# SysCV/LiDAR_snow_sim

Measured on NVIDIA H100. Metric: augmented LiDAR points/sec, higher is better.
Workload: dtype f64

## Files before the change

include/lidar_snow_sim.h:

```cpp
#ifndef LIDAR_SNOW_SIM_H
#define LIDAR_SNOW_SIM_H

#include <stdint.h>

#ifdef __cplusplus
extern "C" {
#endif

#if defined(__GNUC__)
#define LSS_API __attribute__((visibility("default")))
#else
#define LSS_API
#endif

typedef struct lss_engine lss_engine;

typedef enum {
    LSS_OK = 0,
    LSS_ERR_INVALID_ARG = 1,
    LSS_ERR_CUDA = 2,
    LSS_ERR_NO_TABLE = 3,
    LSS_ERR_RANGE_INDEX = 4,
    LSS_ERR_NEGATIVE_INTENSITY = 5,
    LSS_ERR_OCCLUDER_OVERFLOW = 6,
// ... 31 lines not shown
                                       int n_azimuth_buckets, void *stream, int *table_id_out);
LSS_API lss_status lss_free_particles(lss_engine *e, int table_id);
LSS_API lss_status lss_table_info(lss_engine *e, int table_id, int64_t *n_particles, int64_t *n_entries, int64_t *bytes);

LSS_API lss_status lss_snowfall_batch(lss_engine *e, int table_id, const float *d_points, const int64_t *h_cloud_offsets,
                              int n_clouds, const int32_t *h_order, double beam_divergence_deg, const float *d_theta,
                              const double *h_thresh_poly, const double *h_plane_in, const int32_t *h_ymins_in,
                              double noise_floor, uint32_t flags, float *d_out_points,
                              int32_t *d_out_counts, double *d_out_stats, float *d_out_full, int32_t *d_out_perm,
                              int32_t *d_out_nocc, void *d_workspace, int64_t workspace_bytes, void *stream);
LSS_API lss_status lss_snowfall_batch_slots(lss_engine *e, int table_id, const float *d_points,
                                            const int64_t *h_cloud_offsets, const int32_t *d_cloud_counts, int n_clouds,
                                            const int32_t *h_order, double beam_divergence_deg, const float *d_theta,
                                            const double *h_thresh_poly, const double *h_plane_in,
                                            const int32_t *h_ymins_in, double noise_floor, uint32_t flags,
                                            float *d_out_points, int32_t *d_out_counts, double *d_out_stats,
                                            float *d_out_full, int32_t *d_out_perm, int32_t *d_out_nocc,
                                            void *d_workspace, int64_t workspace_bytes, void *stream);
LSS_API int64_t lss_snowfall_workspace_bytes(int64_t n_total, int n_clouds);
LSS_API lss_status lss_snowfall_batch_host(lss_engine *e, int table_id, const float *h_points,
                                           const int64_t *h_cloud_offsets, int n_clouds, const int32_t *h_order,
                                           double beam_divergence_deg, const double *h_thresh_poly, double noise_floor,
                                           uint32_t flags, int n_chunks, float *h_out_points, int32_t *h_out_counts,
                                           double *h_out_stats);
LSS_API lss_status lss_snowfall_batch_host_submit(lss_engine *e, int table_id, const float *h_points,
                                                  const int64_t *h_cloud_offsets, int n_clouds, const int32_t *h_order,
                                                  double beam_divergence_deg, const double *h_thresh_poly,
                                                  double noise_floor, uint32_t flags, int n_chunks, float *h_out_points,
                                                  int32_t *h_out_counts, double *h_out_stats, int *ticket_out);
LSS_API lss_status lss_snowfall_batch_host_wait(lss_engine *e, int ticket);
LSS_API int lss_host_pipe_trace(lss_engine *e, float *out, int cap_chunks);
LSS_API lss_status lss_check_async(lss_engine *e, void *stream);
LSS_API int64_t lss_launch_count(const lss_engine *e);
LSS_API lss_status lss_noise_threshold_poly(lss_engine *e, const float *d_points, const int64_t *h_cloud_offsets,
                                    int n_clouds, double noise_floor, const double *h_plane_in,
                                    const int32_t *h_ymins_in, double *d_poly_out, double *d_plane_out,
                                    double *d_fit_out, int32_t *d_ymins_out, void *d_workspace,
                                    int64_t workspace_bytes, void *stream);
LSS_API int64_t lss_prepass_workspace_bytes(int64_t n_total, int n_clouds);

LSS_API lss_status lss_wet_ground_batch(lss_engine *e, const float *d_points, const int64_t *h_cloud_offsets,
                                const int32_t *d_cloud_counts, int n_clouds, double water_height, double pavement_depth,
                                double noise_floor, double power_factor, int flat_earth, double delta, int replace,
                                const double *h_plane_in, const int32_t *h_ymins_in, float *d_out_points,
                                double *d_out_intensity64, int32_t *d_out_counts, int32_t *d_out_passthrough,
                                double *d_out_plane, double *d_out_fit, int32_t *d_out_ymins, void *d_workspace,
                                int64_t workspace_bytes, void *stream);
LSS_API lss_status lss_wet_ground_batch_params(lss_engine *e, const float *d_points, const int64_t *h_cloud_offsets,
                                               const int32_t *d_cloud_counts, int n_clouds,
                                               const double *h_water_height, double pavement_depth,
                                               double noise_floor, double power_factor, int flat_earth, double delta,
                                               int replace, const double *h_plane_in, const int32_t *h_ymins_in,
                                               float *d_out_points, double *d_out_intensity64, int32_t *d_out_counts,
                                               int32_t *d_out_passthrough, double *d_out_plane, double *d_out_fit,
                                               int32_t *d_out_ymins, void *d_workspace, int64_t workspace_bytes,
                                               void *stream);
LSS_API int64_t lss_wet_ground_workspace_bytes(int64_t n_total, int n_clouds);
LSS_API lss_status lss_wet_ground_batch_poly(lss_engine *e, const float *d_points, const int64_t *h_cloud_offsets,
                                             const int32_t *d_cloud_counts, int n_clouds, const double *h_water_height,
                                             double pavement_depth, double noise_floor, double power_factor,
                                             int flat_earth, double delta, int replace, const double *h_plane_in,
                                             const int32_t *h_ymins_in, const uint32_t *h_mt_state,
                                             float *d_out_points, double *d_out_intensity64, int32_t *d_out_counts,
                                             int32_t *d_out_passthrough, double *d_out_plane, double *d_out_fit,
                                             int32_t *d_out_ymins, uint32_t *d_mt_state_out, double *d_out_poly_fit,
                                             void *d_workspace, int64_t workspace_bytes, void *stream);
// ... 219 lines not shown
```

lidar_snow_sim_b200/_lib.py:

```python
import ctypes
import os

_HERE = os.path.dirname(os.path.abspath(__file__))
LIB_PATH = os.path.join(_HERE, 'liblss_b200.so')

LSS_OK = 0
LSS_ERR_INVALID_ARG = 1
LSS_ERR_CUDA = 2
LSS_ERR_NO_TABLE = 3
LSS_ERR_RANGE_INDEX = 4
LSS_ERR_NEGATIVE_INTENSITY = 5
LSS_ERR_OCCLUDER_OVERFLOW = 6
LSS_ERR_WORKSPACE = 7
LSS_ERR_NO_SENSOR = 8
LSS_ERR_TOO_FEW_GROUND = 9
LSS_ERR_INTENSITY_RANGE = 10

FLAG_THRESHOLD_FILTER = 0x1
FLAG_CAMERA_FOV = 0x2
FLAG_DEVICE_PREPASS = 0x4
FLAG_ASSUME_SORTED = 0x8
FOG_HARD, FOG_SOFT, FOG_GAIN = 0x1, 0x2, 0x4
DROR_CUBE, DROR_WORK_STATS = 0x1, 0x100

# ... 17 lines not shown
    LSS_ERR_TOO_FEW_GROUND: TypeError,
    LSS_ERR_INTENSITY_RANGE: ValueError,
}

_c = ctypes
_P = ctypes.c_void_p
SIGNATURES = [
    ('lss_create', _c.c_int, [_c.c_int, _c.POINTER(_P)]),
    ('lss_destroy', None, [_P]),
    ('lss_status_string', _c.c_char_p, [_c.c_int]),
    ('lss_last_error', _c.c_char_p, [_P]),
    ('lss_version', _c.c_int, []),
    ('lss_set_sensor', _c.c_int, [_P, _c.c_int, _P, _P, _P, _P]),
    ('lss_set_camera', _c.c_int, [_P, _P, _P, _P, _c.c_int, _c.c_int]),
    ('lss_upload_particles', _c.c_int, [_P, _c.c_int, _P, _P, _c.c_double, _c.c_int, _P, _c.POINTER(_c.c_int)]),
    ('lss_upload_particles_device', _c.c_int, [_P, _c.c_int, _P, _P, _c.c_double, _c.c_int, _P,
                                               _c.POINTER(_c.c_int)]),
    ('lss_free_particles', _c.c_int, [_P, _c.c_int]),
    ('lss_table_info', _c.c_int, [_P, _c.c_int, _c.POINTER(_c.c_int64), _c.POINTER(_c.c_int64),
                                  _c.POINTER(_c.c_int64)]),
    ('lss_snowfall_batch', _c.c_int, [_P, _c.c_int, _P, _P, _c.c_int, _P, _c.c_double, _P, _P, _P, _P, _c.c_double,
                                      _c.c_uint32, _P, _P, _P, _P, _P, _P, _P, _c.c_int64, _P]),
    ('lss_snowfall_batch_slots', _c.c_int, [_P, _c.c_int, _P, _P, _P, _c.c_int, _P, _c.c_double, _P, _P, _P, _P,
                                            _c.c_double, _c.c_uint32, _P, _P, _P, _P, _P, _P, _P, _c.c_int64, _P]),
    ('lss_snowfall_workspace_bytes', _c.c_int64, [_c.c_int64, _c.c_int]),
    ('lss_host_pipe_trace', _c.c_int, [_P, _P, _c.c_int]),
    ('lss_snowfall_batch_host', _c.c_int, [_P, _c.c_int, _P, _P, _c.c_int, _P, _c.c_double, _P, _c.c_double, _c.c_uint32,
                                           _c.c_int, _P, _P, _P]),
    ('lss_snowfall_batch_host_submit', _c.c_int, [_P, _c.c_int, _P, _P, _c.c_int, _P, _c.c_double, _P, _c.c_double,
                                                  _c.c_uint32, _c.c_int, _P, _P, _P, _c.POINTER(_c.c_int)]),
    ('lss_snowfall_batch_host_wait', _c.c_int, [_P, _c.c_int]),
    ('lss_check_async', _c.c_int, [_P, _P]),
    ('lss_launch_count', _c.c_int64, [_P]),
    ('lss_debug_range_grid', _c.c_int, [_P]),
    ('lss_debug_azimuth', _c.c_int, [_P, _P, _P, _c.c_int64, _P, _P]),
    ('lss_debug_solve_phases', _c.c_int, [_P, _c.c_int, _P, _c.c_int]),
    ('lss_noise_threshold_poly', _c.c_int, [_P, _P, _P, _c.c_int, _c.c_double, _P, _P, _P, _P, _P, _P, _P, _c.c_int64,
                                            _P]),
    ('lss_prepass_workspace_bytes', _c.c_int64, [_c.c_int64, _c.c_int]),
    ('lss_wet_ground_batch', _c.c_int, [_P, _P, _P, _P, _c.c_int, _c.c_double, _c.c_double, _c.c_double, _c.c_double,
                                        _c.c_int, _c.c_double, _c.c_int, _P, _P, _P, _P, _P, _P, _P, _P, _P, _P,
                                        _c.c_int64, _P]),
    ('lss_wet_ground_batch_params', _c.c_int, [_P, _P, _P, _P, _c.c_int, _P, _c.c_double, _c.c_double, _c.c_double,
                                               _c.c_int, _c.c_double, _c.c_int, _P, _P, _P, _P, _P, _P, _P, _P, _P,
                                               _P, _c.c_int64, _P]),
    ('lss_wet_ground_workspace_bytes', _c.c_int64, [_c.c_int64, _c.c_int]),
    ('lss_wet_ground_batch_poly', _c.c_int, [_P, _P, _P, _P, _c.c_int, _P, _c.c_double, _c.c_double, _c.c_double,
                                             _c.c_int, _c.c_double, _c.c_int, _P, _P, _P, _P, _P, _P, _P, _P, _P, _P,
                                             _P, _P, _P, _c.c_int64, _P]),
    ('lss_wet_ground_poly_workspace_bytes', _c.c_int64, [_c.c_int64, _c.c_int]),
    ('lss_fog_batch', _c.c_int, [_P, _P, _c.c_int, _P, _c.c_int, _c.c_double, _c.c_double, _c.c_double, _P, _c.c_uint32,
                                 _c.c_int, _c.c_int, _P, _P, _P, _P, _P, _P, _P, _c.c_int64, _P]),
    ('lss_fog_workspace_bytes', _c.c_int64, [_c.c_int64, _c.c_int]),
    ('lss_fog_batch_params', _c.c_int, [_P, _P, _c.c_int, _P, _c.c_int, _P, _P, _P, _P, _P, _c.c_int, _c.c_uint32,
                                        _c.c_int, _c.c_int, _P, _P, _P, _P, _P, _P, _P, _c.c_int64, _P]),
    ('lss_fog_batch_params_workspace_bytes', _c.c_int64, [_c.c_int64, _c.c_int]),
    ('lss_fog_integral_tables', _c.c_int, [_P, _P, _c.c_int, _P, _P, _c.c_int64, _P]),
    ('lss_fog_integral_tables_workspace_bytes', _c.c_int64, [_c.c_int, _c.c_int]),
    ('lss_mie_tables', _c.c_int, [_P, _P, _P, _c.c_int, _P, _c.c_int, _P, _P, _c.c_int64, _P]),
    ('lss_mie_tables_workspace_bytes', _c.c_int64, [_P, _P, _c.c_int, _P, _c.c_int]),
    ('lss_lisa_batch', _c.c_int, [_P, _P, _c.c_int, _c.c_int64, _c.c_double, _c.c_int, _c.c_double, _c.c_double, _c.c_double,
                                  _c.c_double, _c.c_double, _c.c_double, _c.c_int, _P, _c.c_int, _c.c_uint64, _P, _P]),
    ('lss_lisa_cloud_batch', _c.c_int, [_P, _P, _c.c_int, _P, _P, _c.c_int, _P, _P, _P, _P, _c.c_int, _c.c_double,
                                        _c.c_double, _c.c_double, _c.c_double, _c.c_double, _c.c_int, _P, _c.c_int, _P, _P,
                                        _P, _P, _c.c_int64, _P]),
    ('lss_lisa_cloud_batch_workspace_bytes', _c.c_int64, [_c.c_int64, _c.c_int]),
# ... 56 lines not shown
                                            _c.c_int64, _P, _c.c_int]),
    ('lss_sample_particles', _c.c_int, [_P, _c.c_int, _c.c_double, _c.c_double, _c.c_double, _c.c_int, _c.c_uint64,
                                        _c.c_int64, _P, _c.c_int64, _P, _P, _P, _c.c_int64, _P]),
    ('lss_sample_particles_workspace_bytes', _c.c_int64, [_c.c_int, _c.c_int64]),
    ('lss_set_profiling', _c.c_int, [_P, _c.c_int]),
    ('lss_kernel_times', _c.c_int, [_P, _c.c_int, _P, _P, _c.c_int]),
    ('lss_kernel_name', _c.c_char_p, [_c.c_int]),
]

_lib = None


def load():
    global _lib
    if _lib is not None:
        return _lib
    if not os.path.exists(LIB_PATH):
        raise ImportError(f'{LIB_PATH} not found: build it with `python -m lidar_snow_sim_b200.build` '
                          f'(or __graft_entry__.build()); this engine has no CPU fallback')
    lib = ctypes.CDLL(LIB_PATH)
    for name, res, args in SIGNATURES:
        fn = getattr(lib, name)
        fn.restype = res
        fn.argtypes = args
    _lib = lib
    return lib


def check(status, engine_handle=None):
    if status == LSS_OK:
        return
    lib = load()
    msg = lib.lss_status_string(status).decode()
    if engine_handle:
        detail = lib.lss_last_error(engine_handle).decode()
        if detail:
            msg = f'{msg}: {detail}'
    raise _EXC.get(status, RuntimeError)(msg)
```

lidar_snow_sim_b200/csrc/api.cu:

```cuda
#include "common.cuh"
#include <cmath>
#include <cstring>
#include <cstdlib>

namespace {

void host_range_grid(double *R)
{
    const double stop = 120 + 299792458.0 * 1e-8;
    const double step = stop / (LSS_M_EXT - 1);
    for (int k = 0; k < LSS_M_EXT; k++) {
        double v = (k == LSS_M_EXT - 1) ? stop : k * step;
        R[k] = std::nearbyint(v * 100.0) / 100.0;
    }
}

void host_phase_table(const double *R, double *tab )
{
    const long double ctau = (long double)(299792458.0 * 1e-8);
    const long double pi = 3.14159265358979323846264338327950288L;
    for (int k = 0; k < LSS_M_EXT; k++) {
        const long double a = fmodl((long double)R[k] / ctau, 2.0L);
        tab[2 * k] = (double)sinl(pi * a);
        tab[2 * k + 1] = (double)cosl(pi * a);
    }
}

}

extern "C" {

int lss_version(void) { return 100; }

const char *lss_status_string(lss_status s)
{
    switch (s) {
        case LSS_OK: return "ok";
        case LSS_ERR_INVALID_ARG: return "invalid argument";
        case LSS_ERR_CUDA: return "CUDA error";
        case LSS_ERR_NO_TABLE: return "particle table set not found";
        case LSS_ERR_RANGE_INDEX: return "waveform index out of range (return beyond ~120 m on an occluded beam)";
        case LSS_ERR_NEGATIVE_INTENSITY: return "new intensity is negative";
        case LSS_ERR_OCCLUDER_OVERFLOW: return "too many occluders on one beam";
        case LSS_ERR_WORKSPACE: return "workspace too small";
        case LSS_ERR_NO_SENSOR: return "sensor / camera constants not set";
        case LSS_ERR_TOO_FEW_GROUND: return "fewer than 3 ground points: laser parameters cannot be estimated";
        case LSS_ERR_INTENSITY_RANGE:
            return "intensity histogram range (5, max(I/cos)) of the ground points is not finite or max is below 5";
    }
    return "unknown status";
}

const char *lss_last_error(const lss_engine *e) { return e ? e->last_error.c_str() : "null engine"; }

lss_status lss_create(int device, lss_engine **out)
{
    if (!out) return LSS_ERR_INVALID_ARG;
    *out = nullptr;
    int n_dev = 0;
    if (cudaGetDeviceCount(&n_dev) != cudaSuccess || n_dev == 0) return LSS_ERR_CUDA;
    if (device < 0 || device >= n_dev) return LSS_ERR_INVALID_ARG;
    lss_engine *e = new lss_engine();
    e->device = device;
    DeviceGuard g(device);
    double R[LSS_M_EXT];
    host_range_grid(R);
    std::vector<double> wtab(2 * LSS_M_EXT);
    host_phase_table(R, wtab.data());
    int zero = 0;
    cudaDeviceGetAttribute(&e->n_sm, cudaDevAttrMultiProcessorCount, device);
    if (e->n_sm <= 0) e->n_sm = 132;
    if (cudaMalloc(&e->d_R, sizeof(R)) != cudaSuccess || cudaMalloc(&e->d_status, sizeof(int)) != cudaSuccess ||
        cudaMalloc(&e->d_wtab, sizeof(double) * wtab.size()) != cudaSuccess ||
        cudaMemcpy(e->d_wtab, wtab.data(), sizeof(double) * wtab.size(), cudaMemcpyHostToDevice) != cudaSuccess ||
        cudaMalloc(&e->d_sensor, sizeof(SensorConst)) != cudaSuccess ||
        cudaMalloc(&e->d_camera, sizeof(CameraConst)) != cudaSuccess ||
        cudaMemcpy(e->d_R, R, sizeof(R), cudaMemcpyHostToDevice) != cudaSuccess ||
        cudaMemcpy(e->d_status, &zero, sizeof(int), cudaMemcpyHostToDevice) != cudaSuccess) {
        lss_destroy(e);
        return LSS_ERR_CUDA;
    }
    *out = e;
    return LSS_OK;
}

void lss_destroy(lss_engine *e)
{
    if (!e) return;
    DeviceGuard g(e->device);
    for (auto &kv : e->tables) {
        cudaFree(kv.second.d_rec);
        cudaFree(kv.second.d_tan);
        cudaFree(kv.second.d_plane_off);
        cudaFree(kv.second.d_entries);
        cudaFree(kv.second.d_bucket_start);
    }
    cudaFree(e->d_R);
    cudaFree(e->d_wtab);
    cudaFree(e->d_status);
    cudaFree(e->d_sensor);
    cudaFree(e->d_camera);
    lss_host_pipe_free(e);
    for (cudaStream_t st : e->side) if (st) { cudaStreamSynchronize(st); cudaStreamDestroy(st); }
    for (cudaEvent_t ev : e->side_ev) if (ev) cudaEventDestroy(ev);
    for (auto &sl : e->stage) {
        if (sl.done) { cudaEventSynchronize(sl.done); cudaEventDestroy(sl.done); }
        if (sl.host) cudaFreeHost(sl.host);
    }
    delete e;
}

// ... 289 lines not shown
```

lidar_snow_sim_b200/csrc/common.cuh:

```cuda
#pragma once
#include <cuda_runtime.h>
#include <stdint.h>
#include <stdio.h>
#include <string>
#include <vector>
#include <cstring>
#include <map>
#include <utility>

#include "../../include/lidar_snow_sim.h"

#define LSS_PI 3.141592653589793
#define LSS_TWO_PI 6.283185307179586
#define LSS_M_EXT 1230
#define LSS_ANG_MARGIN 1e-5

struct ParticleRec {
    double phi;
    double rho;
    double alpha;
};
struct ParticleTan {
    double t_right, t_left;
};
// ... 248 lines not shown
       LSS_K_FOG = 6, LSS_K_SCAN = 7, LSS_K_SOLVE = 8, LSS_K_VOXEL = 9, LSS_K_DROR = 10, LSS_K_LISA = 11,
       LSS_K_FOG_LUT = 12, LSS_K_MIE = 13, LSS_K_SELECT = 14, LSS_K_PA = 15, LSS_K_COUNT = 16 };

struct KernelTimer {
    lss_engine *e; cudaStream_t s; int idx = -1;
    KernelTimer(lss_engine *e_, int kernel, cudaStream_t s_) : e(e_), s(s_) {
        if (!e->profiling) return;
        lss_engine::TimedLaunch t; t.kernel = kernel;
        cudaEventCreate(&t.beg); cudaEventCreate(&t.end);
        cudaEventRecord(t.beg, s);
        e->timed.push_back(t); idx = (int)e->timed.size() - 1;
    }
    ~KernelTimer() { if (idx >= 0) cudaEventRecord(e->timed[idx].end, s); }
};

#define LSS_CUDA_CHECK(e, call)                                                                          \
    do {                                                                                                 \
        cudaError_t _err = (call);                                                                       \
        if (_err != cudaSuccess) {                                                                       \
            char _buf[512];                                                                              \
            snprintf(_buf, sizeof(_buf), "%s failed: %s (%s:%d)", #call, cudaGetErrorString(_err),      \
                     __FILE__, __LINE__);                                                                \
            (e)->last_error = _buf;                                                                      \
            return LSS_ERR_CUDA;                                                                         \
        }                                                                                                \
    } while (0)

struct DeviceGuard {
    int prev = -1;
    explicit DeviceGuard(int dev) { cudaGetDevice(&prev); if (prev != dev) cudaSetDevice(dev); else prev = -1; }
    ~DeviceGuard() { if (prev >= 0) cudaSetDevice(prev); }
};

static inline lss_status lss_fail(lss_engine *e, lss_status s, const char *msg)
{
    if (e) e->last_error = msg;
    return s;
}

struct BatchGeometry {
    int64_t n = 0, max_n = 0;
    std::vector<int32_t> tile_base;
};

inline lss_status lss_batch_geometry(lss_engine *e, const int64_t *h_cloud_offsets, int n_clouds, int tile,
                                     BatchGeometry &g)
{
    if (!h_cloud_offsets || n_clouds < 0) return lss_fail(e, LSS_ERR_INVALID_ARG, "null argument");
    if (n_clouds > 65535) return lss_fail(e, LSS_ERR_INVALID_ARG, "at most 65535 clouds per call");
    if (h_cloud_offsets[0] != 0) return lss_fail(e, LSS_ERR_INVALID_ARG, "cloud_offsets[0] must be 0");
    g.max_n = 0;
    g.tile_base.assign(tile > 0 ? n_clouds + 1 : 0, 0);
    for (int b = 0; b < n_clouds; b++) {
        const int64_t n = h_cloud_offsets[b + 1] - h_cloud_offsets[b];
        if (n < 0) return lss_fail(e, LSS_ERR_INVALID_ARG, "cloud_offsets must be non-decreasing");
        if (n >= (1LL << 31)) return lss_fail(e, LSS_ERR_INVALID_ARG, "cloud too large");
        g.max_n = n > g.max_n ? n : g.max_n;
        if (tile > 0) g.tile_base[b + 1] = g.tile_base[b] + (int32_t)((n + tile - 1) / tile);
    }
    g.n = h_cloud_offsets[n_clouds];
    return LSS_OK;
}

lss_status lss_build_tables(lss_engine *e, TableSet &ts, const double *d_xyr, const int64_t *h_plane_offsets,
                            cudaStream_t stream);
struct SnowfallArgs {
// ... 82 lines not shown
```

lidar_snow_sim_b200/csrc/solve.cu:

```cuda
#include "beam.cuh"

namespace {

constexpr int SOLVE_TPB = 128;
constexpr int SOLVE_WARPS = SOLVE_TPB / 32;
#ifndef LSS_SOLVE_CTAS
#define LSS_SOLVE_CTAS 5
#endif
#ifndef LSS_SOLVE_ARENA
#define LSS_SOLVE_ARENA 160
#endif
constexpr int SOLVE_CTAS_PER_SM = LSS_SOLVE_CTAS;
constexpr int ARENA = LSS_SOLVE_ARENA;
constexpr int SOLVE_LCAP = 128;
static_assert(SOLVE_LCAP + 1 <= ARENA, "a beam with SOLVE_LCAP occluders must fit a round of the arena on its own");
constexpr unsigned FULL = 0xffffffffu;

struct Beam {
    double d, right, left;
    bool straddle;
};

__device__ __forceinline__ void beam_limits(float th32, double half_div, Beam &bm)
{
    const double thd = (double)th32;
    double right = thd - half_div, left = thd + half_div;
    if (right < 0) right += LSS_TWO_PI;
    if (left < 0) left += LSS_TWO_PI;
    if (right > LSS_TWO_PI) right -= LSS_TWO_PI;
    if (left > LSS_TWO_PI) left -= LSS_TWO_PI;
    bm.right = right; bm.left = left; bm.straddle = right > left;
}

__device__ __forceinline__ bool exact_hit(const ParticleRec *rp, const Beam &bm, double &rho, bool &right_hit, bool &left_hit)
{
    rho = rp->rho;
    const double phi = rp->phi, alpha = rp->alpha;
    bool inside = (bm.right <= phi) & (phi <= bm.left);
    if (bm.straddle) inside = inside | ((bm.right - LSS_TWO_PI <= phi) & (phi <= bm.left)) |
                              ((bm.right <= phi) & (phi <= bm.left + LSS_TWO_PI));
// ... 221 lines not shown
        a.keep_tag[beg + i] = (uint8_t)ch;
    }
    __syncwarp();
    {
        float *dst = a.aug + (beg + w0) * 5;
#pragma unroll
        for (int q = 0; q < 5; q++) {
            const int f = q * 32 + lane;
            if (f < nf_w) dst[f] = s_rows[wid][f];
        }
    }
}

__device__ __forceinline__ unsigned long long pack_win(int ks, int ke, int k0)
{
    return (unsigned long long)(unsigned)ks | ((unsigned long long)(unsigned)ke << 11) | ((unsigned long long)(unsigned)k0 << 22);
}

__device__ __forceinline__ void pulse_phase(double r, double &sb, double &cb)
{
    const double ctau = 299792458.0 * 1e-8, inv_ctau = 1.0 / (299792458.0 * 1e-8);
    const double bh = r * inv_ctau;
    const double bl = fma(-bh, ctau, r) * inv_ctau;
    double s, c;
    sincospi(bh, &s, &c);
    const double corr = LSS_PI * bl;
    sb = fma(corr, c, s);
    cb = fma(-corr, s, c);
}

__device__ __forceinline__ void cp_async8(void *dst, const void *src)
{
    asm volatile("cp.async.ca.shared.global [%0], [%1], 8;\n" ::"r"((unsigned)__cvta_generic_to_shared(dst)), "l"(src) : "memory");
}
__device__ __forceinline__ void cp_async_wait_all() { asm volatile("cp.async.wait_all;\n" ::: "memory"); }

#ifdef LSS_SOLVE_PHASE_CLOCKS
enum { PH_FETCH, PH_FILL, PH_CLAIM, PH_PULSES, PH_SWEEP, PH_EVAL, PH_STORE, PH_N };
static_assert(PH_N + 2 + LIST_CLASSES == LSS_DEBUG_SOLVE_PHASE_WORDS, "layout of lss_debug_solve_phases");
__device__ unsigned long long g_solve_phase[LSS_DEBUG_SOLVE_PHASE_WORDS];
#define PHASE_INIT()                                                                                                  \
    __shared__ unsigned long long s_ph[SOLVE_WARPS][PH_N + 1];                                                        \
    if (lane <= PH_N) s_ph[wid][lane] = 0ull;                                                                         \
    unsigned ph_t = (unsigned)clock64();                         \
    unsigned ph_split = 0u
#define PHASE(k)                                                                                                      \
    do {                                                                                                              \
        const unsigned ph_n = (unsigned)clock64();                                                                    \
        if (lane == 0) s_ph[wid][k] += ph_n - ph_t;                                                                   \
        ph_t = ph_n;                                                                                                  \
    } while (0)
#define PHASE_MARK() (ph_split = (unsigned)clock64() - ph_t)
#define PHASE_SPLIT(k0, k1)                                                                                           \
    do {                                                                                                              \
        const unsigned ph_n = (unsigned)clock64();                                                                    \
        const unsigned sp = __reduce_max_sync(FULL, ph_split);                                                        \
        if (lane == 0) { s_ph[wid][k0] += sp; s_ph[wid][k1] += ph_n - ph_t - sp; }                                   \
        ph_t = ph_n;                                                                                                  \
        ph_split = 0u;                                                                                                \
    } while (0)
#define PHASE_TILE(cls, active)                                                                                       \
    do {                                                                                                              \
        const unsigned nb = __popc(__ballot_sync(FULL, active));                                                      \
        if (lane == 0) { s_ph[wid][PH_N]++; atomicAdd(&g_solve_phase[PH_N + 2 + (cls)], (unsigned long long)nb); }    \
    } while (0)
#define PHASE_FLUSH()                                                                                                 \
    do {                                                                                                              \
        if (lane <= PH_N) atomicAdd(&g_solve_phase[lane], s_ph[wid][lane]);                                           \
        if (lane == 0) atomicAdd(&g_solve_phase[PH_N + 1], 1ull);                                                     \
    } while (0)
#else
#define PHASE_INIT()
#define PHASE(k)
#define PHASE_MARK()
#define PHASE_SPLIT(k0, k1)
#define PHASE_TILE(cls, active)
#define PHASE_FLUSH()
#endif

__global__ void __launch_bounds__(SOLVE_TPB, SOLVE_CTAS_PER_SM) k_solve(DevArgs a, int *tile_cursor)
{
    __shared__ double s_arena[SOLVE_WARPS][4][ARENA];
    __shared__ unsigned long long s_piece[SOLVE_WARPS][2 * ARENA];
    __shared__ int s_piece_k[SOLVE_WARPS][2 * ARENA];
    const int lane = threadIdx.x & 31, wid = threadIdx.x >> 5;
    unsigned long long *PD = s_piece[wid];
    int *PK = s_piece_k[wid];
    double *A0 = s_arena[wid][0], *A1 = s_arena[wid][1], *A2 = s_arena[wid][2], *A3 = s_arena[wid][3];
    unsigned long long *W = reinterpret_cast<unsigned long long *>(A2);

    __shared__ int s_tile0[LIST_CLASSES + 1];
    __shared__ int s_cnt[LIST_CLASSES];
    lss_pdl_trigger();
    lss_pdl_wait();
    if (wid == 0) {
        int run = 0;
        for (int c0 = 0; c0 < LIST_CLASSES; c0 += 32) {
            const int n = a.hdr[LIST_CLASSES + c0 + lane];
            s_cnt[c0 + lane] = n;
            const int v = (n + 31) >> 5;
            int incl = v;
#pragma unroll
            for (int sft = 1; sft < 32; sft <<= 1) {
                const int t = __shfl_up_sync(FULL, incl, sft);
                if (lane >= sft) incl += t;
            }
            s_tile0[c0 + lane] = run + incl - v;
            run += __shfl_sync(FULL, incl, 31);
        }
        if (lane == 0) s_tile0[LIST_CLASSES] = run;
    }
    __syncthreads();
    const int n_tiles = s_tile0[LIST_CLASSES];
    const double ctau = 299792458.0 * 1e-8;
    const double inv_step = (double)(LSS_M_EXT - 1) / (120 + ctau);
    PHASE_INIT();

    const auto beam_of = [&](int t, int &c, int &j) {
        c = 0;
#pragma unroll
        for (int step = LIST_CLASSES / 2; step; step >>= 1)
            if (s_tile0[c + step] <= t) c += step;
        j = (t - s_tile0[c]) * 32 + lane;
        return t < n_tiles && j < s_cnt[c];
    };
    const auto chunk_of = [&](int c, int j) { return a.chunk_tab[(int64_t)c * a.chunks_per_class + j / LIST_CHUNK]; };
    const auto item_of = [&](int chunk, int j) { return a.items[(int64_t)(chunk - 1) * LIST_CHUNK + j % LIST_CHUNK]; };
    const auto empty_item = [] {
        SolveItem e;
        e.key = 0ull; e.hit_off = 0; e.L = 0; e.th32 = 0.0f; e.px = 0.0f; e.py = 0.0f; e.pz = 0.0f;
        return e;
    };
    int tile = 0;
    if (lane == 0) tile = atomicAdd(tile_cursor, 1);
    tile = __shfl_sync(FULL, tile, 0);
    SolveItem it = empty_item();
    {
        int c, j;
        if (beam_of(tile, c, j)) it = item_of(chunk_of(c, j), j);
    }

    while (tile < n_tiles) {
        int cls, jn;
        const bool active = beam_of(tile, cls, jn);
        int nxt = 0;
        if (lane == 0) nxt = atomicAdd(tile_cursor, 1);
        int nchunk = 0;
        bool fetched = false;
        SolveItem nx = empty_item();
        const auto next_chunk = [&] {
            nxt = __shfl_sync(FULL, nxt, 0);
            if (beam_of(nxt, cls, jn)) nchunk = chunk_of(cls, jn);
        };
        const auto next_item = [&] {
            if (nchunk > 0) nx = item_of(nchunk, jn);
            fetched = true;
        };
        const int b = (int)((it.key >> 32) & 0xffffu);
        const int i = (int)(it.key & 0xffffffffu);
        const int ch = (int)(it.key >> 56);
        const int64_t beg = a.cloud_off[b];
        const float px = it.px, py = it.py, pz = it.pz;
        const float d32 = __fsqrt_rn(__fadd_rn(__fadd_rn(__fmul_rn(px, px), __fmul_rn(py, py)), __fmul_rn(pz, pz)));

        float out_x = px, out_y = py, out_z = pz, out_i = 0.0f, out_l = 0.0f;
        long long att_new_i = -1;
        int n_claim = 0;

        const int L = active ? it.L : 0;
        Beam bm;
        bm.d = (double)d32;
        beam_limits(it.th32, a.half_div, bm);

        if (L > SOLVE_LCAP) raise_status(a.status, LSS_ERR_OCCLUDER_OVERFLOW);
        const int need = (L > 0 && L <= SOLVE_LCAP) ? L + 1 : 0;
        PHASE_TILE(cls, active);
        PHASE(PH_FETCH);

        unsigned remaining = __ballot_sync(FULL, need > 0);
        while (remaining) {
            const bool rem = (remaining >> lane) & 1u;
            const int mine = rem ? need : 0;
            int incl = mine;
#pragma unroll
            for (int s = 1; s < 32; s <<= 1) {
                const int t = __shfl_up_sync(FULL, incl, s);
                if (lane >= s) incl += t;
            }
            const bool in_round = rem && incl <= ARENA;
            remaining &= ~__ballot_sync(FULL, in_round);
            const int off = incl - mine;
            const int total = (int)__reduce_max_sync(FULL, in_round ? (unsigned)incl : 0u);
            int n_pulses = 0;
            double amax = 0.0;
            double best = 0.0;
            int kbest = 0;

#pragma unroll 1
            for (int s0 = 0; s0 < total; s0 += 32) {
                const int s = s0 + lane;
                int j = 0;
#pragma unroll
                for (int step = 16; step; step >>= 1) {
                    const int c = j + step;
                    const int oc = __shfl_sync(FULL, off, c & 31);
                    if (c < 32 && oc <= s) j = c;
                }
                const int r = s - __shfl_sync(FULL, off, j);
                const int Lj = __shfl_sync(FULL, L, j);
                const int hoj = __shfl_sync(FULL, it.hit_off, j);
                const int inr = __shfl_sync(FULL, (int)in_round, j);
                if (s < total && inr && r < Lj && hoj >= 0) {
                    cp_async8(&A0[s], &a.hit_a1[hoj + r]);
                    cp_async8(&A1[s], &a.hit_a2[hoj + r]);
                    cp_async8(&A2[s], &a.hit_rho[hoj + r]);
                }
            }
            cp_async_wait_all();
            __syncwarp();
            if (in_round && it.hit_off < 0) {
                const Bucket bkt = beam_bucket(a, a.order[b * LSS_N_CHANNELS + ch], it.th32);
                int s = off;
                for_each_hit(a, bkt, bm, d32, [&](int pi, double rho, bool rh, bool lh) {
                    A0[s] = rh ? bm.right : a.tan[pi].t_right;
                    A1[s] = lh ? bm.left : a.tan[pi].t_left;
                    A2[s] = rho;
                    s++;
                });
            }
            __syncwarp();
            if (!fetched) next_chunk();
            PHASE(PH_FILL);

            if (in_round) {
#pragma unroll 1
                for (int p = 1; p < L; p++) {
                    const double rho = A2[off + p];
                    if (!(A2[off + p - 1] > rho)) continue;
                    const double a1 = A0[off + p], a2 = A1[off + p];
                    int q = p - 1;
#pragma unroll 1
                    while (q >= 0 && A2[off + q] > rho) { A0[off + q + 1] = A0[off + q]; A1[off + q + 1] = A1[off + q]; A2[off + q + 1] = A2[off + q]; q--; }
                    A0[off + q + 1] = a1; A1[off + q + 1] = a2; A2[off + q + 1] = rho;
                }

                double rb = bm.right;
                if (bm.straddle) rb = bm.right - LSS_TWO_PI;
                int nu = 0, P = 0;
                double ep_min = fmin(rb, bm.left), ep_max = fmax(rb, bm.left), claimed_total = 0.0;
#pragma unroll 1
                for (int j = 0; j < L; j++) {
                    double lo = A0[off + j];
                    const double hi = A1[off + j], rho = A2[off + j];
                    if (bm.straddle && lo > hi) lo -= LSS_TWO_PI;
                    ep_min = fmin(ep_min, fmin(lo, hi));
                    ep_max = fmax(ep_max, fmax(lo, hi));
                    if (!(lo < hi)) continue;
                    bool contained = false;
                    double cov = 0.0, nlo = lo, nhi = hi;
                    int w = 0;
#pragma unroll 1
                    for (int u = 0; u < nu; u++) {
                        const double ul = A0[off + u], uh = A1[off + u];
                        if ((ul <= lo) && (hi <= uh)) { contained = true; break; }
                        if (ul <= hi && uh >= lo) {
                            const double ov = fmin(hi, uh) - fmax(lo, ul);
                            if (ov > 0.0) cov += ov;
                            nlo = fmin(nlo, ul);
                            nhi = fmax(nhi, uh);
                        } else {
                            A0[off + w] = ul; A1[off + w] = uh; w++;
                        }
                    }
                    if (contained) continue;
                    const double claimed = (hi - lo) - cov;
                    claimed_total += claimed;
                    A0[off + w] = nlo; A1[off + w] = nhi;
                    nu = w + 1;
// ... 12 lines not shown
                    const double beta_0 = 1 * 1e-06 / LSS_PI;
                    const double i_orig = 0.9 * a.sensor->max_intensity[ch];
                    const double A = (i_orig / beta_0) * beta_0;
                    bool bad = false;
#pragma unroll 1
                    for (int j = 0; j < P; j++) {
                        const double r = A2[off + j], ratio = A3[off + j];
                        const int ks = (int)ceil(r * 10);
                        const int ke = (int)(floor((r + ctau) * 10) + 1);
                        bad |= (ke > LSS_M_EXT) || (ks < 0);
                        double sb, cb;
                        pulse_phase(r, sb, cb);
                        const double amp = (A * ratio * xsi64(r)) / (r * r);
                        amax = fmax(amax, amp);
                        A0[off + j] = amp;
                        A1[off + j] = sb;
                        A3[off + j] = cb;
                        W[off + j] = pack_win(ks, ke, (int)rint((r + ctau / 2) * inv_step));
                    }
                    {
                        const int ks = (int)ceilf(__fmul_rn(d32, 10.0f));
                        const int ke = (int)(floorf(__fmul_rn(__fadd_rn(d32, (float)ctau), 10.0f)) + 1.0f);
                        bad |= (ke > LSS_M_EXT) || (ks < 0);
                        double sb, cb;
                        pulse_phase(bm.d, sb, cb);
                        const double amp = (A * ratio_hard * xsi32(d32)) / (double)__fmul_rn(d32, d32);
                        amax = fmax(amax, amp);
                        A0[off + P] = amp;
                        A1[off + P] = sb;
                        A3[off + P] = cb;
                        W[off + P] = pack_win(ks, ke, (int)rint((bm.d + ctau / 2) * inv_step));
                    }
                    if (bad) raise_status(a.status, LSS_ERR_RANGE_INDEX);
                    else n_pulses = P + 1;
                }
            }
            PHASE_SPLIT(PH_CLAIM, PH_PULSES);
            if (!fetched) next_item();

            int np_mine = 0;
            if (n_pulses > 0) {
                const double lb = 0.99 * amax;
                double asum = 0.0;
                int qa = 0, qb = -1, nxt = 0;
                int ks_n = (int)(W[off] & 2047u);
                int ke_a = 0;
                int k = ks_n;
                unsigned long long *pd = PD + 2 * off;
#pragma unroll 1
                for (;;) {
#pragma unroll 1
                    while (ks_n <= k) {
                        qb = nxt++;
                        asum += A0[off + qb];
                        ks_n = nxt < n_pulses ? (int)(W[off + nxt] & 2047u) : 4096;
                    }
#pragma unroll 1
                    while (qa <= qb) {
                        ke_a = (int)((W[off + qa] >> 11) & 2047u);
                        if (ke_a > k) break;
                        asum -= A0[off + qa];
                        qa++;
                    }
                    if (qa > qb) {
                        asum = 0.0;
                        if (nxt >= n_pulses) break;
                        k = ks_n;
// ... 52 lines not shown
                            kc = (int)((W[qa] >> 22) & 2047u);
                        } else {
                            float zx = 0.0f, zy = 0.0f, asum = 0.0f;
#pragma unroll 1
                            for (int q = qa; q <= qb; q++) {
                                const float A = (float)A0[q], sn = (float)A1[q], cs = (float)A3[q];
                                zx += A * (cs * cs - sn * sn);
                                zy += A * (2.0f * sn * cs);
                                asum += A;
                            }
                            all = zx * zx + zy * zy < 1e-6f * asum * asum;
                            const float r0 = (atan2f(zy, zx) + 3.14159265f) * (ctau_f * 0.15915494f);
                            const float rc = 0.5f * (float)(lo + hi - 1) * step;
                            kc = (int)rintf((r0 + rintf((rc - r0) / ctau_f) * ctau_f) / step);
                        }
                        const int c_lo = all ? lo : max(lo, min(hi - 1, kc - 1));
                        const int c_hi = all ? hi - 1 : min(hi - 1, max(lo, kc + 1));
#pragma unroll 1
                        for (int c = c_lo; c <= c_hi; c++) eval(c);
                        PD[slot] = (unsigned long long)__double_as_longlong(pbest);
                        PK[slot] = pk;
                    }
                }
            }
            __syncwarp();
#pragma unroll 1
            for (int r = 0; r < np_mine; r++) {
                const double v = __longlong_as_double((long long)PD[2 * off + r]);
                if (v > best) { best = v; kbest = PK[2 * off + r]; }
            }
            __syncwarp();
            PHASE(PH_EVAL);

            if (n_pulses > 0) {
                const double max_i = a.sensor->max_intensity[ch];
                const double min_i = a.sensor->min_intensity[ch];
                const double d_max = ((double)kbest / 10) - (ctau / 2);
                const double q1 = 1 - d_max / 120;
                double i_max = best + max_i * a.sensor->focal_slope[ch] * fabs(a.sensor->focal_offset[ch] - q1 * q1);
                i_max = i_max < min_i ? min_i : (i_max > max_i ? max_i : i_max);
                const long long new_i = (long long)i_max;
                if (fabs(d_max - bm.d) < 2 * (1.0 / 10)) {
                    out_l = 1.0f;
                    att_new_i = new_i;
                } else {
                    out_l = 2.0f;
                    const double sc = d_max / bm.d;
                    out_x = (float)((double)px * sc);
                    out_y = (float)((double)py * sc);
                    out_z = (float)((double)pz * sc);
                }
                if (new_i < 0) raise_status(a.status, LSS_ERR_NEGATIVE_INTENSITY);
                double ci = (double)new_i;
                ci = ci < min_i ? min_i : (ci > max_i ? max_i : ci);
                out_i = (float)ci;
            }
            __syncwarp();
            PHASE(PH_STORE);
        }
        if (!fetched) { next_chunk(); next_item(); }

        if (active) {
            if (out_l != 0.0f) {
                const float ri = rintf(out_i);
                float *row = a.aug + (beg + i) * 5;
                row[0] = out_x; row[1] = out_y; row[2] = out_z; row[3] = ri; row[4] = out_l;
                a.keep_i[beg + i] = ri;
                a.keep_tag[beg + i] = keep_tag_of(ch, out_l);
            }
            if (a.nocc) a.nocc[beg + i] = n_claim;
        }
        {
            const bool on = att_new_i >= 0;
            const int key = b * LSS_N_CHANNELS + (ch < LSS_N_CHANNELS ? ch : 0);
            const unsigned mk = __match_any_sync(FULL, on ? key : -1);
            if (on && lane == __ffs(mk) - 1) atomicAdd(a.att_cnt + key, (unsigned)__popc(mk));
            const unsigned mb = __match_any_sync(FULL, on ? b : -1);
            const unsigned sum = __reduce_add_sync(mb, on ? (unsigned)att_new_i : 0u);
            if (on && lane == __ffs(mb) - 1) atomicAdd(&a.att_sum[b], (unsigned long long)sum);
        }
        PHASE(PH_STORE);
        tile = nxt;
        it = nx;
    }
    PHASE_FLUSH();
}

}

namespace {
__global__ void k_debug_azimuth(const float *y, const float *x, float *out, int64_t n)
{
    const int64_t i = (int64_t)blockIdx.x * blockDim.x + threadIdx.x;
    if (i < n) out[i] = azimuth32(y[i], x[i]);
}
}

extern "C" lss_status lss_debug_azimuth(lss_engine *e, const float *d_y, const float *d_x, int64_t n, float *d_out, void *stream)
{
    if (!e || !d_y || !d_x || !d_out || n < 0) return LSS_ERR_INVALID_ARG;
    if (n == 0) return LSS_OK;
    DeviceGuard g(e->device);
    LSS_CUDA_CHECK(e, lss_launch(e, k_debug_azimuth, (unsigned)((n + 255) / 256), 256, 0, (cudaStream_t)stream, d_y, d_x,
                                 d_out, n));
    return LSS_OK;
}

extern "C" lss_status lss_debug_solve_phases(lss_engine *e, int reset, uint64_t *h_out, int n)
{
    if (!e || (h_out && n < LSS_DEBUG_SOLVE_PHASE_WORDS)) return LSS_ERR_INVALID_ARG;
#ifdef LSS_SOLVE_PHASE_CLOCKS
    DeviceGuard g(e->device);
    LSS_CUDA_CHECK(e, cudaDeviceSynchronize());
    if (h_out) LSS_CUDA_CHECK(e, cudaMemcpyFromSymbol(h_out, g_solve_phase, sizeof(g_solve_phase)));
    if (reset) {
        static const unsigned long long zero[LSS_DEBUG_SOLVE_PHASE_WORDS] = {};
        LSS_CUDA_CHECK(e, cudaMemcpyToSymbol(g_solve_phase, zero, sizeof(zero)));
    }
    return LSS_OK;
#else
    (void)reset;
    return lss_fail(e, LSS_ERR_INVALID_ARG, "lss_debug_solve_phases: the library was built without -DLSS_SOLVE_PHASE_CLOCKS");
#endif
}

#ifndef LSS_PDL_SOLVE
#define LSS_PDL_SOLVE 1
#endif
cudaError_t lss_launch_scan(lss_engine *e, const DevArgs &a, cudaStream_t stream)
{
    return lss_launch_pdl(e, k_scan, (unsigned)((a.n_wtiles + SNOW_WARPS - 1) / SNOW_WARPS), SNOW_TPB, 0, stream, a);
}

cudaError_t lss_launch_solve(lss_engine *e, const DevArgs &a, int *tile_cursor, cudaStream_t stream)
{
    const unsigned grid = (unsigned)(e->n_sm * SOLVE_CTAS_PER_SM);
    if (LSS_PDL_SOLVE) return lss_launch_pdl(e, k_solve, grid, SOLVE_TPB, 0, stream, a, tile_cursor);
    return lss_launch(e, k_solve, grid, SOLVE_TPB, 0, stream, a, tile_cursor);
}
```

lidar_snow_sim_b200/engine.py:

```python
import ctypes
import math

import numpy as np
import torch

from . import _lib
from .calib.hdl64e_s3 import sensor_arrays

DEFAULT_MAX_DIVERGENCE_RAD = 3e-3
SAMPLER_ATTEMPTS = 4
LISA_SEED_STATE = np.random.RandomState(666).get_state()
MAX_CLOUDS = 65535
_CPU = torch.device('cpu')


def _ptr(t):
    if t is None:
        return None
    if isinstance(t, torch.Tensor):
        return ctypes.c_void_p(t.data_ptr())
    if isinstance(t, np.ndarray):
        return ctypes.c_void_p(t.ctypes.data)
    raise TypeError(type(t))

# ... 847 lines not shown
        if need < 0:
            raise ValueError('bad cloud_offsets')
        ws = self._scratch('gt_paste', need)
        out = torch.empty((int(n_out), F), dtype=torch.float32, device=self.device)
        out_counts = torch.empty((B,), dtype=torch.int32, device=self.device)
        self._call('lss_gt_paste_batch', points, F, _ptr(off), counts, B, rm_boxes, rm_offsets, int(max_rm), ops,
                   ops.shape[1], db, objects, object_shift, objects.shape[0], int(n_object_rows), out_offsets,
                   object_rows, out, out_counts, ws, ws.numel())
        return out, out_counts

    def gather_push(self, points, counts, d_cloud_offsets, n_rows, world, rank, peer_points, peer_counts, mc_points=0,
                    mc_counts=0, blocks=0):
        _check_tensor('d_cloud_offsets', d_cloud_offsets, self.device, torch.int64, (None,))
        B = d_cloud_offsets.shape[0] - 1
        _check_tensor('points', points, self.device, torch.float32, (None, 5))
        _check_tensor('counts', counts, self.device, torch.int32, (B,), optional=True)
        peer_points, peer_counts, world = list(peer_points), list(peer_counts), int(world)
        if len(peer_points) != world or len(peer_counts) != world:
            raise ValueError(f'peer_points / peer_counts: {len(peer_points)} / {len(peer_counts)} buffers for {world} ranks')
        for r in range(world):
            _check_tensor(f'peer_points[{r}]', peer_points[r], None, torch.float32, (world * int(n_rows), 5))
            _check_tensor(f'peer_counts[{r}]', peer_counts[r], None, torch.int32, (world * B,))
        P = ctypes.c_void_p * world
        self._call('lss_gather_push', points, counts, d_cloud_offsets, B, int(n_rows), world, int(rank),
                   P(*[t.data_ptr() for t in peer_points]), P(*[t.data_ptr() for t in peer_counts]), mc_points or None,
                   mc_counts or None, int(blocks))

    def check(self):
        self._call('lss_check_async')

    def launch_count(self):
        return int(self.lib.lss_launch_count(self.h))

    def set_profiling(self, enable=True):
        _lib.check(self.lib.lss_set_profiling(self.h, 1 if enable else 0), self.h)

    def kernel_times(self, reset=True):
        torch.cuda.synchronize(self.device)
        n = 16
        ms = np.zeros(n, dtype=np.float64)
        calls = np.zeros(n, dtype=np.int64)
        _lib.check(self.lib.lss_kernel_times(self.h, 1 if reset else 0, _ptr(ms), _ptr(calls), n), self.h)
        names = [self.lib.lss_kernel_name(k).decode() for k in range(n)]
        return {names[k]: (float(ms[k]), int(calls[k])) for k in range(n) if names[k]}


_default_engines = {}


def default_engine(device=None):
    if device is None:
        device = torch.cuda.current_device() if torch.cuda.is_available() else 0
    if device not in _default_engines:
        _default_engines[device] = SnowfallEngine(device)
    return _default_engines[device]
```

Baseline: 5.086 billion.

## Raise solve kernel CTAs per SM, shrink per-beam state, prefetch items via cp.async

The persistent solve kernel now launches six CTAs per SM instead of five. To make that fit, it shrinks shared and register footprint: piece indices become uint16, the output point coordinates are recomputed at store time instead of being carried through the loop, and beam limits are recomputed where needed. The next work item is prefetched as an int4 register load plus a 16-byte cp.async into shared memory, replacing a whole SolveItem held in registers. A create-time occupancy check fails if the persistent grid cannot be fully resident, which adds a correctness guard but also a new failure mode.

```diff
diff --git a/include/lidar_snow_sim.h b/include/lidar_snow_sim.h
--- a/include/lidar_snow_sim.h
+++ b/include/lidar_snow_sim.h
@@ -87,6 +87,7 @@
 LSS_API int lss_host_pipe_trace(lss_engine *e, float *out, int cap_chunks);
 LSS_API lss_status lss_check_async(lss_engine *e, void *stream);
 LSS_API int64_t lss_launch_count(const lss_engine *e);
+LSS_API lss_status lss_solve_ctas_per_sm(lss_engine *e, int *launched, int *resident);
 LSS_API lss_status lss_noise_threshold_poly(lss_engine *e, const float *d_points, const int64_t *h_cloud_offsets,
                                     int n_clouds, double noise_floor, const double *h_plane_in,
                                     const int32_t *h_ymins_in, double *d_poly_out, double *d_plane_out,
diff --git a/lidar_snow_sim_b200/_lib.py b/lidar_snow_sim_b200/_lib.py
--- a/lidar_snow_sim_b200/_lib.py
+++ b/lidar_snow_sim_b200/_lib.py
@@ -73,6 +73,7 @@
     ('lss_snowfall_batch_host_wait', _c.c_int, [_P, _c.c_int]),
     ('lss_check_async', _c.c_int, [_P, _P]),
     ('lss_launch_count', _c.c_int64, [_P]),
+    ('lss_solve_ctas_per_sm', _c.c_int, [_P, _c.POINTER(_c.c_int), _c.POINTER(_c.c_int)]),
     ('lss_debug_range_grid', _c.c_int, [_P]),
     ('lss_debug_azimuth', _c.c_int, [_P, _P, _P, _c.c_int64, _P, _P]),
     ('lss_debug_solve_phases', _c.c_int, [_P, _c.c_int, _P, _c.c_int]),
@@ -195,8 +196,7 @@
         return
     lib = load()
     msg = lib.lss_status_string(status).decode()
-    if engine_handle:
-        detail = lib.lss_last_error(engine_handle).decode()
-        if detail:
-            msg = f'{msg}: {detail}'
+    detail = lib.lss_last_error(engine_handle).decode()
+    if detail:
+        msg = f'{msg}: {detail}'
     raise _EXC.get(status, RuntimeError)(msg)
diff --git a/lidar_snow_sim_b200/csrc/api.cu b/lidar_snow_sim_b200/csrc/api.cu
--- a/lidar_snow_sim_b200/csrc/api.cu
+++ b/lidar_snow_sim_b200/csrc/api.cu
@@ -51,12 +51,15 @@
     return "unknown status";
 }
 
-const char *lss_last_error(const lss_engine *e) { return e ? e->last_error.c_str() : "null engine"; }
+static thread_local std::string t_create_error;
+
+const char *lss_last_error(const lss_engine *e) { return e ? e->last_error.c_str() : t_create_error.c_str(); }
 
 lss_status lss_create(int device, lss_engine **out)
 {
     if (!out) return LSS_ERR_INVALID_ARG;
     *out = nullptr;
+    t_create_error.clear();
     int n_dev = 0;
     if (cudaGetDeviceCount(&n_dev) != cudaSuccess || n_dev == 0) return LSS_ERR_CUDA;
     if (device < 0 || device >= n_dev) return LSS_ERR_INVALID_ARG;
@@ -77,6 +80,19 @@
         cudaMalloc(&e->d_camera, sizeof(CameraConst)) != cudaSuccess ||
         cudaMemcpy(e->d_R, R, sizeof(R), cudaMemcpyHostToDevice) != cudaSuccess ||
         cudaMemcpy(e->d_status, &zero, sizeof(int), cudaMemcpyHostToDevice) != cudaSuccess) {
+        lss_destroy(e);
+        return LSS_ERR_CUDA;
+    }
+    int launched = 0, resident = 0;
+    const cudaError_t ce = lss_solve_occupancy(&launched, &resident);
+    if (ce != cudaSuccess || resident != launched) {
+        char buf[256];
+        if (ce != cudaSuccess)
+            snprintf(buf, sizeof(buf), "solve kernel occupancy query failed: %s", cudaGetErrorString(ce));
+        else
+            snprintf(buf, sizeof(buf), "the solve kernel's persistent grid needs %d CTAs per SM resident, the device holds %d",
+                     launched, resident);
+        t_create_error = buf;
         lss_destroy(e);
         return LSS_ERR_CUDA;
     }
diff --git a/lidar_snow_sim_b200/csrc/common.cuh b/lidar_snow_sim_b200/csrc/common.cuh
--- a/lidar_snow_sim_b200/csrc/common.cuh
+++ b/lidar_snow_sim_b200/csrc/common.cuh
@@ -304,6 +304,8 @@
     ~DeviceGuard() { if (prev >= 0) cudaSetDevice(prev); }
 };
 
+cudaError_t lss_solve_occupancy(int *launched, int *resident);
+
 static inline lss_status lss_fail(lss_engine *e, lss_status s, const char *msg)
 {
     if (e) e->last_error = msg;
diff --git a/lidar_snow_sim_b200/csrc/solve.cu b/lidar_snow_sim_b200/csrc/solve.cu
--- a/lidar_snow_sim_b200/csrc/solve.cu
+++ b/lidar_snow_sim_b200/csrc/solve.cu
@@ -5,7 +5,7 @@
 constexpr int SOLVE_TPB = 128;
 constexpr int SOLVE_WARPS = SOLVE_TPB / 32;
 #ifndef LSS_SOLVE_CTAS
-#define LSS_SOLVE_CTAS 5
+#define LSS_SOLVE_CTAS 6
 #endif
 #ifndef LSS_SOLVE_ARENA
 #define LSS_SOLVE_ARENA 160
@@ -293,6 +293,10 @@
 __device__ __forceinline__ void cp_async8(void *dst, const void *src)
 {
     asm volatile("cp.async.ca.shared.global [%0], [%1], 8;\n" ::"r"((unsigned)__cvta_generic_to_shared(dst)), "l"(src) : "memory");
+}
+__device__ __forceinline__ void cp_async16(void *dst, const void *src)
+{
+    asm volatile("cp.async.cg.shared.global [%0], [%1], 16;\n" ::"r"((unsigned)__cvta_generic_to_shared(dst)), "l"(src) : "memory");
 }
 __device__ __forceinline__ void cp_async_wait_all() { asm volatile("cp.async.wait_all;\n" ::: "memory"); }
 
@@ -343,10 +347,11 @@
 {
     __shared__ double s_arena[SOLVE_WARPS][4][ARENA];
     __shared__ unsigned long long s_piece[SOLVE_WARPS][2 * ARENA];
-    __shared__ int s_piece_k[SOLVE_WARPS][2 * ARENA];
+    __shared__ uint16_t s_piece_k[SOLVE_WARPS][2 * ARENA];
+    __shared__ __align__(16) float4 s_item[SOLVE_WARPS][32];
     const int lane = threadIdx.x & 31, wid = threadIdx.x >> 5;
     unsigned long long *PD = s_piece[wid];
-    int *PK = s_piece_k[wid];
+    uint16_t *PK = s_piece_k[wid];
     double *A0 = s_arena[wid][0], *A1 = s_arena[wid][1], *A2 = s_arena[wid][2], *A3 = s_arena[wid][3];
     unsigned long long *W = reinterpret_cast<unsigned long long *>(A2);
 
@@ -386,19 +391,18 @@
         return t < n_tiles && j < s_cnt[c];
     };
     const auto chunk_of = [&](int c, int j) { return a.chunk_tab[(int64_t)c * a.chunks_per_class + j / LIST_CHUNK]; };
-    const auto item_of = [&](int chunk, int j) { return a.items[(int64_t)(chunk - 1) * LIST_CHUNK + j % LIST_CHUNK]; };
-    const auto empty_item = [] {
-        SolveItem e;
-        e.key = 0ull; e.hit_off = 0; e.L = 0; e.th32 = 0.0f; e.px = 0.0f; e.py = 0.0f; e.pz = 0.0f;
-        return e;
+    int4 nh = make_int4(0, 0, 0, 0);
+    const auto fetch_item = [&](int chunk, int j) {
+        const SolveItem *src = a.items + (int64_t)(chunk - 1) * LIST_CHUNK + j % LIST_CHUNK;
+        nh = *reinterpret_cast<const int4 *>(src);
+        cp_async16(&s_item[wid][lane], reinterpret_cast<const char *>(src) + 16);
     };
     int tile = 0;
     if (lane == 0) tile = atomicAdd(tile_cursor, 1);
     tile = __shfl_sync(FULL, tile, 0);
-    SolveItem it = empty_item();
     {
         int c, j;
-        if (beam_of(tile, c, j)) it = item_of(chunk_of(c, j), j);
+        if (beam_of(tile, c, j)) fetch_item(chunk_of(c, j), j);
     }
 
     while (tile < n_tiles) {
@@ -408,30 +412,42 @@
         if (lane == 0) nxt = atomicAdd(tile_cursor, 1);
         int nchunk = 0;
         bool fetched = false;
-        SolveItem nx = empty_item();
         const auto next_chunk = [&] {
             nxt = __shfl_sync(FULL, nxt, 0);
             if (beam_of(nxt, cls, jn)) nchunk = chunk_of(cls, jn);
         };
         const auto next_item = [&] {
-            if (nchunk > 0) nx = item_of(nchunk, jn);
+            if (nchunk > 0) fetch_item(nchunk, jn);
             fetched = true;
         };
+        SolveItem it;
+        cp_async_wait_all();
+        if (active) {
+            it.key = (unsigned long long)(unsigned)nh.x | ((unsigned long long)(unsigned)nh.y << 32);
+            it.hit_off = nh.z; it.L = nh.w;
+            const float4 q = s_item[wid][lane];
+            it.th32 = q.x; it.px = q.y; it.py = q.z; it.pz = q.w;
+        } else {
+            it.key = 0ull; it.hit_off = 0; it.L = 0; it.th32 = 0.0f; it.px = 0.0f; it.py = 0.0f; it.pz = 0.0f;
+        }
         const int b = (int)((it.key >> 32) & 0xffffu);
         const int i = (int)(it.key & 0xffffffffu);
         const int ch = (int)(it.key >> 56);
-        const int64_t beg = a.cloud_off[b];
         const float px = it.px, py = it.py, pz = it.pz;
         const float d32 = __fsqrt_rn(__fadd_rn(__fadd_rn(__fmul_rn(px, px), __fmul_rn(py, py)), __fmul_rn(pz, pz)));
 
-        float out_x = px, out_y = py, out_z = pz, out_i = 0.0f, out_l = 0.0f;
-        long long att_new_i = -1;
+        bool solved = false;
+        double best = 0.0;
+        int kbest = 0;
         int n_claim = 0;
 
         const int L = active ? it.L : 0;
-        Beam bm;
-        bm.d = (double)d32;
-        beam_limits(it.th32, a.half_div, bm);
+        const auto limits = [&] {
+            Beam bm;
+            bm.d = (double)d32;
+            beam_limits(it.th32, a.half_div, bm);
+            return bm;
+        };
 
         if (L > SOLVE_LCAP) raise_status(a.status, LSS_ERR_OCCLUDER_OVERFLOW);
         const int need = (L > 0 && L <= SOLVE_LCAP) ? L + 1 : 0;
@@ -454,8 +470,6 @@
             const int total = (int)__reduce_max_sync(FULL, in_round ? (unsigned)incl : 0u);
             int n_pulses = 0;
             double amax = 0.0;
-            double best = 0.0;
-            int kbest = 0;
 
 #pragma unroll 1
             for (int s0 = 0; s0 < total; s0 += 32) {
@@ -481,6 +495,7 @@
             __syncwarp();
             if (in_round && it.hit_off < 0) {
                 const Bucket bkt = beam_bucket(a, a.order[b * LSS_N_CHANNELS + ch], it.th32);
+                const Beam bm = limits();
                 int s = off;
                 for_each_hit(a, bkt, bm, d32, [&](int pi, double rho, bool rh, bool lh) {
                     A0[s] = rh ? bm.right : a.tan[pi].t_right;
@@ -505,6 +520,7 @@
                     A0[off + q + 1] = a1; A1[off + q + 1] = a2; A2[off + q + 1] = rho;
                 }
 
+                const Beam bm = limits();
                 double rb = bm.right;
                 if (bm.straddle) rb = bm.right - LSS_TWO_PI;
                 int nu = 0, P = 0;
@@ -583,7 +599,7 @@
                         W[off + P] = pack_win(ks, ke, (int)rint((bm.d + ctau / 2) * inv_step));
                     }
                     if (bad) raise_status(a.status, LSS_ERR_RANGE_INDEX);
-                    else n_pulses = P + 1;
+                    else { n_pulses = P + 1; solved = true; }
                 }
             }
             PHASE_SPLIT(PH_CLAIM, PH_PULSES);
@@ -702,39 +718,46 @@
             __syncwarp();
             PHASE(PH_EVAL);
 
-            if (n_pulses > 0) {
-                const double max_i = a.sensor->max_intensity[ch];
-                const double min_i = a.sensor->min_intensity[ch];
-                const double d_max = ((double)kbest / 10) - (ctau / 2);
-                const double q1 = 1 - d_max / 120;
-                double i_max = best + max_i * a.sensor->focal_slope[ch] * fabs(a.sensor->focal_offset[ch] - q1 * q1);
-                i_max = i_max < min_i ? min_i : (i_max > max_i ? max_i : i_max);
-                const long long new_i = (long long)i_max;
-                if (fabs(d_max - bm.d) < 2 * (1.0 / 10)) {
-                    out_l = 1.0f;
-                    att_new_i = new_i;
-                } else {
-                    out_l = 2.0f;
-                    const double sc = d_max / bm.d;
-                    out_x = (float)((double)px * sc);
-                    out_y = (float)((double)py * sc);
-                    out_z = (float)((double)pz * sc);
-                }
-                if (new_i < 0) raise_status(a.status, LSS_ERR_NEGATIVE_INTENSITY);
-                double ci = (double)new_i;
-                ci = ci < min_i ? min_i : (ci > max_i ? max_i : ci);
-                out_i = (float)ci;
-            }
             __syncwarp();
             PHASE(PH_STORE);
         }
         if (!fetched) { next_chunk(); next_item(); }
 
+        float out_i = 0.0f, out_l = 0.0f;
+        double sc = 1.0;
+        long long att_new_i = -1;
+        if (solved) {
+            const double max_i = a.sensor->max_intensity[ch];
+            const double min_i = a.sensor->min_intensity[ch];
+            const double d_max = ((double)kbest / 10) - (ctau / 2);
+            const double q1 = 1 - d_max / 120;
+            double i_max = best + max_i * a.sensor->focal_slope[ch] * fabs(a.sensor->focal_offset[ch] - q1 * q1);
+            i_max = i_max < min_i ? min_i : (i_max > max_i ? max_i : i_max);
+            const long long new_i = (long long)i_max;
+            if (fabs(d_max - (double)d32) < 2 * (1.0 / 10)) {
+                out_l = 1.0f;
+                att_new_i = new_i;
+            } else {
+                out_l = 2.0f;
+                sc = d_max / (double)d32;
+            }
+            if (new_i < 0) raise_status(a.status, LSS_ERR_NEGATIVE_INTENSITY);
+            double ci = (double)new_i;
+            ci = ci < min_i ? min_i : (ci > max_i ? max_i : ci);
+            out_i = (float)ci;
+        }
+
         if (active) {
+            const int64_t beg = a.cloud_off[b];
             if (out_l != 0.0f) {
                 const float ri = rintf(out_i);
                 float *row = a.aug + (beg + i) * 5;
-                row[0] = out_x; row[1] = out_y; row[2] = out_z; row[3] = ri; row[4] = out_l;
+                if (out_l == 2.0f) {
+                    row[0] = (float)((double)px * sc);
+                    row[1] = (float)((double)py * sc);
+                    row[2] = (float)((double)pz * sc);
+                }
+                row[3] = ri; row[4] = out_l;
                 a.keep_i[beg + i] = ri;
                 a.keep_tag[beg + i] = keep_tag_of(ch, out_l);
             }
@@ -751,7 +774,6 @@
         }
         PHASE(PH_STORE);
         tile = nxt;
-        it = nx;
     }
     PHASE_FLUSH();
 }
@@ -802,6 +824,22 @@
     return lss_launch_pdl(e, k_scan, (unsigned)((a.n_wtiles + SNOW_WARPS - 1) / SNOW_WARPS), SNOW_TPB, 0, stream, a);
 }
 
+cudaError_t lss_solve_occupancy(int *launched, int *resident)
+{
+    cudaError_t ce = cudaFuncSetAttribute(k_solve, cudaFuncAttributePreferredSharedMemoryCarveout, cudaSharedmemCarveoutMaxShared);
+    if (ce == cudaSuccess) ce = cudaOccupancyMaxActiveBlocksPerMultiprocessor(resident, k_solve, SOLVE_TPB, 0);
+    *launched = SOLVE_CTAS_PER_SM;
+    return ce;
+}
+
+extern "C" lss_status lss_solve_ctas_per_sm(lss_engine *e, int *launched, int *resident)
+{
+    if (!e || !launched || !resident) return LSS_ERR_INVALID_ARG;
+    DeviceGuard g(e->device);
+    LSS_CUDA_CHECK(e, lss_solve_occupancy(launched, resident));
+    return LSS_OK;
+}
+
 cudaError_t lss_launch_solve(lss_engine *e, const DevArgs &a, int *tile_cursor, cudaStream_t stream)
 {
     const unsigned grid = (unsigned)(e->n_sm * SOLVE_CTAS_PER_SM);
diff --git a/lidar_snow_sim_b200/engine.py b/lidar_snow_sim_b200/engine.py
--- a/lidar_snow_sim_b200/engine.py
+++ b/lidar_snow_sim_b200/engine.py
@@ -903,6 +903,11 @@
     def launch_count(self):
         return int(self.lib.lss_launch_count(self.h))
 
+    def solve_ctas_per_sm(self):
+        launched, resident = ctypes.c_int(), ctypes.c_int()
+        _lib.check(self.lib.lss_solve_ctas_per_sm(self.h, ctypes.byref(launched), ctypes.byref(resident)), self.h)
+        return launched.value, resident.value
+
     def set_profiling(self, enable=True):
         _lib.check(self.lib.lss_set_profiling(self.h, 1 if enable else 0), self.h)
 
```

New measurement: 5.154 billion, median of 6. 1.01x the previous value.
